# jmloveyj/ros_navigation

Measured on AMD Instinct MI355X. Metric: replan cycles/sec (HIMM+VFH++A*) on 4096x4096 grid, higher is better.
Workload: dtype int32; 1 GPU; full replan loop on 4096x4096 f32 grid (res 0.05 m); one step = one turn of the 20-stage A* pipeline = 20 passes of [100032-ray HIMM batch + fused compose -> 256 VFH+ poses -> 256 grid-A* queries (one launch)]; 30% rectangle obstacles (seed 2); 4 ray batches / pose sets / query sets in rotation; cycles_per_pass=256, rays_per_pass=100032, rotating_input_sets=4, astar_queries_checked=15360, astar_queries_answered=15360, astar_bucket_width=128000, astar_pipeline_depth=20, parallelism=query-sharded x1, full=False

## Files before the change

ros_navigation_amd/csrc/astar_tile.hip:

```cpp
#include "engine.hpp"
#include <algorithm>
#include <cstring>
#include <vector>

using namespace rna;

namespace rna {

constexpr int TI = 64, TJ = 16;
constexpr int TILE_WORDS = TI * TJ;
constexpr int AUX_WORDS = 64;
constexpr int MASK_STRIDE = TILE_WORDS + 32 + 128;
constexpr int TSA_WAVES = 8;
constexpr int TSA_WAVES_PER_EU = 8;
constexpr int TSA_HPASS = 4;
constexpr int TSA_IDLE_SLEEP = 4;
constexpr int TSA_PRIO_FIRST = 0;
constexpr int TSA_BT_PRIO = 3;
constexpr int TSA_SCOPE = __HIP_MEMORY_SCOPE_AGENT;
constexpr int TSA_MAX_TILE_WORDS = 2048;
constexpr int COST_S = 1000, COST_D = 1414;
constexpr int INF = 0x7fffffff;
constexpr int KU = 0x40000000;
constexpr int SCR_CNT = 84 + 192 + 48 + 64;
// ... 70 lines not shown

__device__ __forceinline__ int tile_of(int i, int j, int tiles_i) { return (j >> 4) * tiles_i + (i >> 6); }
__device__ __forceinline__ int in_page(int i, int j) { return ((j & 15) << 6) + (i & 63); }
__device__ __forceinline__ int kdi_of(int k) { return (k == 0 || k == 3 || k == 5) ? -1 : ((k == 2 || k == 4 || k == 7) ? 1 : 0); }
__device__ __forceinline__ int kdj_of(int k) { return k < 3 ? -1 : (k > 4 ? 1 : 0); }

struct TsaStage {
  unsigned* pages;
  unsigned* paux;
  unsigned* tmap;
  unsigned* owner;
  int* nalloc;
  uint8_t* nbr_tm;
  int* perm;
  int* ticket;
  int cap;
};
__host__ __device__ inline size_t tsa_align256(size_t x) { return (x + 255) & ~(size_t)255; }
constexpr int TSA_COUNTER_WORDS = 16;
__host__ __device__ inline unsigned long long* tsa_counters_of(const TsaStage& S) {
  return reinterpret_cast<unsigned long long*>(reinterpret_cast<char*>(S.nalloc) - TSA_COUNTER_WORDS * sizeof(unsigned long long));
}

__global__ void __launch_bounds__(256) tsa_snapshot_kernel(const uint8_t* __restrict__ nbr, int rows, int cols, int tiles_i, int tiles_j,
                                                             uint8_t* __restrict__ nbr_tm, int s0, int s1) {
  __shared__ unsigned s_free[256];
  const int a = threadIdx.x & 63, bq = threadIdx.x >> 6;
  for (int t = blockIdx.x; t < tiles_i * tiles_j; t += gridDim.x) {
    const int i = (t % tiles_i) * TI + a, j0 = (t / tiles_i) * TJ + bq * 4;
    unsigned v = 0u;
    if (i < rows) {
      const int bi = i + s0 >= rows ? i + s0 - rows : i + s0;
#pragma unroll
      for (int k = 0; k < 4; ++k)
        if (j0 + k < cols) {
          const int bj = j0 + k + s1 >= cols ? j0 + k + s1 - cols : j0 + k + s1;
          v |= (unsigned)nbr[(size_t)bj * rows + bi] << (8 * k);
        }
    }
    uint8_t* out = nbr_tm + (size_t)t * MASK_STRIDE;
    reinterpret_cast<unsigned*>(out)[a * 4 + bq] = v;
    if (a == 0) reinterpret_cast<unsigned*>(out + TILE_WORDS)[bq] = v;
    if (a == TI - 1) reinterpret_cast<unsigned*>(out + TILE_WORDS + 16)[bq] = v;
    s_free[threadIdx.x] = (((v & 0xffu) != 0u) ? 1u : 0u) | (((v & 0xff00u) != 0u) ? 2u : 0u) | (((v & 0xff0000u) != 0u) ? 4u : 0u) |
                          (((v & 0xff000000u) != 0u) ? 8u : 0u);
    __syncthreads();
    if (bq == 0)
      reinterpret_cast<unsigned short*>(out + TILE_WORDS + 32)[a] =
          (unsigned short)(s_free[a] | (s_free[64 + a] << 4) | (s_free[128 + a] << 8) | (s_free[192 + a] << 12));
    __syncthreads();
  }
}
__global__ void __launch_bounds__(256) tsa_prepare_kernel(TsaStage S, const rna_astar_query* __restrict__ queries, int n, int rows, int cols,
                                                          int ranked, int* __restrict__ served) {
  extern __shared__ int s_key[];
  if (threadIdx.x == 0) *S.ticket = 0;
  if (served && threadIdx.x < TSA_RETRY) served[threadIdx.x] = -1;
  if (served && threadIdx.x == TSA_RETRY) served[TSA_RETRY] = 0;
  if (!ranked) {
    for (int i = threadIdx.x; i < n; i += blockDim.x) S.perm[i] = i;
    return;
  }
  const int ncell = rows * cols;
  for (int i = threadIdx.x; i < n; i += blockDim.x) {
    const rna_astar_query q = queries[i];
    int key = -1;
    if (q.start >= 0 && q.goal >= 0 && q.start < ncell && q.goal < ncell) {
      const int di = abs(q.start % rows - q.goal % rows), dj = abs(q.start / rows - q.goal / rows);
      key = di > dj ? di : dj;
    }
    s_key[i] = key;
  }
  __syncthreads();
  for (int i = threadIdx.x; i < n; i += blockDim.x) {
    const int ki = s_key[i];
    int rank = 0;
    for (int j = 0; j < n; ++j) {
      const int kj = s_key[j];
      rank += (kj > ki || (kj == ki && j < i)) ? 1 : 0;
    }
    S.perm[rank] = i;
  }
}
__global__ void tsa_fill_pages_kernel(uint4* __restrict__ p, size_t n4) {
  const size_t step = (size_t)gridDim.x * blockDim.x;
  for (size_t w = (size_t)blockIdx.x * blockDim.x + threadIdx.x; w < n4; w += step) p[w] = make_uint4(0u, 0u, 0u, 0u);
}

#ifdef RNA_TSA_STATS
__device__ unsigned long long g_tsa_stat[32];
#define TSA_T(var) const unsigned long long var = wall_clock64()
#define TSA_ACC(slot, t0, t1) tsa_acc[slot] += (unsigned long long)((t1) - (t0))
#define TSA_CNT(slot, v) tsa_acc[slot] += (unsigned long long)(v)
#define TSA_ACC_PARAM , unsigned long long* tsa_acc
#define TSA_ACC_ARG , tsa_acc
#else
#define TSA_ACC_PARAM
#define TSA_ACC_ARG
#define TSA_T(var)
#define TSA_ACC(slot, t0, t1)
#define TSA_CNT(slot, v)
#endif

constexpr int TSA_NCLS = 256;
constexpr int TSA_NP = 3072;
constexpr int TSA_BMW = TSA_NP / 32;
constexpr int TSA_QC = 1024;
constexpr unsigned POP_EMPTY = 0xffffffffu;
static_assert(TSA_NP % 32 == 0 && TSA_NP < 0xffff, "node indices are 16 bits, 0xffff = none");
static_assert(TSA_NP * 4 >= (TI + 2) * (TJ + 2) * 4 + TILE_WORDS, "the backtrace's LDS image lives in the queue memory");

__device__ __forceinline__ unsigned lds_ld(const unsigned* p) { return __hip_atomic_load(p, __ATOMIC_RELAXED, __HIP_MEMORY_SCOPE_WORKGROUP); }
__device__ __forceinline__ int lds_ldi(const int* p) { return __hip_atomic_load(p, __ATOMIC_RELAXED, __HIP_MEMORY_SCOPE_WORKGROUP); }

struct TsaLocalSched {
  int* best_;
  int* state_;
  unsigned* st2_;
  unsigned* far_;
  unsigned* node_;
  unsigned* head_;
  unsigned* bm_;
  unsigned* qc_;
  int* count_;
  int* spill_;
  unsigned* open_;
  int* open_left_;
  __device__ __forceinline__ int best() const { return __hip_atomic_load(best_, __ATOMIC_RELAXED, __HIP_MEMORY_SCOPE_WORKGROUP); }
  __device__ __forceinline__ void improve_best(int g) { atomicMin(best_, g); }
  __device__ __forceinline__ void overflow() { *state_ = 4; }
  __device__ __forceinline__ void pool_exhausted() { *state_ = 5; }
  __device__ __forceinline__ void act_far(int t) { atomicOr(&far_[t >> 5], 1u << (t & 31)); }
  __device__ __forceinline__ bool is_far(int t) const { return (lds_ld(&far_[t >> 5]) >> (t & 31)) & 1u; }
  __device__ __forceinline__ int node_alloc(unsigned seed) {
    unsigned w = ((seed & 0xffffu) * (unsigned)TSA_BMW) >> 16;
    for (int tries = 0; tries < 32; ++tries) {
      const unsigned v = lds_ld(&bm_[w]);
      if (v) {
        const unsigned b = v & (0u - v);
        if (atomicAnd(&bm_[w], ~b) & b) return (int)(w * 32u) + __builtin_ctz(b);
      } else {
        w = w + 1u == (unsigned)TSA_BMW ? 0u : w + 1u;
      }
    }
    return -1;
  }
  __device__ __forceinline__ void node_free(int idx) { atomicOr(&bm_[idx >> 5], 1u << (idx & 31)); }
  __device__ __forceinline__ void link(int idx, unsigned t, unsigned cls) {
    for (;;) {
      const unsigned hv = lds_ld(&head_[cls]);
      __hip_atomic_store(&node_[idx], (hv << 16) | t, __ATOMIC_RELAXED, __HIP_MEMORY_SCOPE_WORKGROUP);
      asm volatile("" ::: "memory");
      if (atomicCAS(&head_[cls], hv, ((hv + 0x10000u) & 0xffff0000u) | (unsigned)idx) == hv) break;
    }
  }
  __device__ __forceinline__ void push(unsigned t, unsigned cls, int lane, int* spare) {
    if (lane == 0) {
      const int idx = *spare >= 0 ? *spare : node_alloc(t * 29u);
      if (idx >= 0) {
        link(idx, t, cls);
        atomicAdd(count_, 1);
        __hip_atomic_store(&qc_[t & (unsigned)(TSA_QC - 1)], (t << 8) | cls, __ATOMIC_RELAXED, __HIP_MEMORY_SCOPE_WORKGROUP);
      } else {
        atomicOr(&far_[t >> 5], 1u << (t & 31));
        *spill_ = 1;
      }
    }
    *spare = -1;
  }
// ... 436 lines not shown
                \
      unsigned long long hsrc_ = up_ & __builtin_amdgcn_ballot_w64(m_ > (mv_ & open_));                          \
      asm volatile("" : "+s"(hsrc_));           \
      const int ht_ = TSA_HT(b);                                                 \
      TSA_G(b) = max(TSA_G(b), m_);                                                                              \
      TSA_PP(b) = TSA_G(b) >= ht_ ? TSA_G(b) : 0;                                                                \
                                                            \
      unsigned left_ = 1u << (TSA_HPASS - 1);                                                                  \
      {                                                                                                          \
        int t1_, t2_;                                                                                            \
        asm volatile(                                                                                            \
            "s_nop 1\n"         \
            ".Lhp_top%=:\n\t"                                                                                     \
            "v_add_u32_dpp %[t1], %[pp], %[nS] wave_shr:1 row_mask:0xf bank_mask:0xf bound_ctrl:1\n\t"             \
            "v_add_u32_dpp %[t2], %[pp], %[nS] wave_shl:1 row_mask:0xf bank_mask:0xf bound_ctrl:1\n\t"             \
            "v_max_i32 %[t1], %[t1], %[t2]\n\t"                                                                   \
            "v_and_b32 %[t1], %[t1], %[open]\n\t"                                                                 \
            "v_cmp_gt_i32 vcc, %[t1], %[g]\n\t"                                                                   \
            "s_cbranch_vccz .Lhp_done%=\n\t"                                                                      \
            "v_max_i32 %[g], %[g], %[t1]\n\t"                                                                     \
            "s_or_b64 %[all], %[all], vcc\n\t"                                                                    \
            "v_cmp_ge_i32 vcc, %[g], %[ht]\n\t"                                                                   \
            "s_nop 1\n\t"                                                                                         \
            "v_cndmask_b32 %[pp], 0, %[g], vcc\n\t"                                                               \
            "s_lshr_b32 %[left], %[left], 1\n\t"                                                                  \
            "s_cbranch_scc1 .Lhp_top%=\n\t"                                                                       \
            ".Lhp_done%=:"                                                                                        \
            : [g] "+v"(TSA_G(b)), [pp] "+v"(TSA_PP(b)), [all] "+s"(up_), [left] "+s"(left_),                       \
              [t1] "=&v"(t1_), [t2] "=&v"(t2_)                                                                   \
            : [nS] "v"(nS), [open] "v"(open_), [ht] "v"(ht_)                                                     \
            : "vcc", "scc");                                                                                     \
      }                                                                                                          \
      TSA_STAT_HP(left_);                                                                                        \
      if (TSA_UNLIKELY(left_ == 0u)) {    \
        if (scan_ok) {                                                                                           \
          TSA_CNT(14, 1);                                                                                        \
          up_ |= tsa_row_fixpoint(TSA_G(b), TSA_PP(b), open_, ht_, thr, lane);                                   \
        } else {                                                                                                 \
          AGVAR |= 1u << (b);                                                                                    \
        }                                                                                                        \
      }                                                                                                          \
      TSA_ROW_CHANGED(b, up_, DIR, hsrc_, left_)                                                                 \
    }                                                                                                            \
  }
#define TSA_DOWN(b) if ((nd >> (b)) & 1u) { nd &= ~(1u << (b)); TSA_ROW(b, TSA_VERT(b, TSA_CAT(TSA_DEC_, b), 0, 2), nu, 0) }
#define TSA_UP(b) if ((nu >> (b)) & 1u) { nu &= ~(1u << (b)); TSA_ROW(b, TSA_VERT(b, TSA_CAT(TSA_INC_, b), 5, 7), nd, 1) }
  for (;;) {
    if (nd != 0u) {
      if (nd & 0x000fu) {
        if (nd & 1u) { nd &= ~1u; TSA_ROW(0, 0, nu, 0) }
        TSA_DOWN(1) TSA_DOWN(2) TSA_DOWN(3)
      }
      if (nd & 0x00f0u) { TSA_DOWN(4) TSA_DOWN(5) TSA_DOWN(6) TSA_DOWN(7) }
      if (nd & 0x0f00u) { TSA_DOWN(8) TSA_DOWN(9) TSA_DOWN(10) TSA_DOWN(11) }
      if (nd & 0xf000u) { TSA_DOWN(12) TSA_DOWN(13) TSA_DOWN(14) TSA_DOWN(15) }
    }
    if (!(nd | nu)) break;
    if (nu != 0u) {
      if (nu & 0xf000u) {
        if ((nu >> 15) & 1u) { nu &= ~(1u << 15); TSA_ROW(15, 0, nd, 1) }
        TSA_UP(14) TSA_UP(13) TSA_UP(12)
      }
      if (nu & 0x0f00u) { TSA_UP(11) TSA_UP(10) TSA_UP(9) TSA_UP(8) }
      if (nu & 0x00f0u) { TSA_UP(7) TSA_UP(6) TSA_UP(5) TSA_UP(4) }
      if (nu & 0x000fu) { TSA_UP(3) TSA_UP(2) TSA_UP(1) TSA_UP(0) }
    }
    if (!(nd | nu)) break;
  }
#undef TSA_DOWN
#undef TSA_UP
#undef TSA_ROW
#undef TSA_VERT
#undef TSA_STAT_INC
#undef TSA_STAT_HP
  TSA_T(t_c);
  TSA_ACC(1, t_b, t_c);
  TSA_CNT(8, evals);
  TSA_CNT(11, hpass);
  if (first) { TSA_CNT(18, 1); TSA_CNT(19, evals); TSA_CNT(20, __builtin_popcount(rowchg)); }
  TSA_CNT(21, __builtin_popcount(rowchg));
  asm volatile("; TSA_MARK results_begin");
  asm volatile("" : "+v"(lane));
  if (rowchg) {
    if (TSA_UNLIKELY(pg == 0u)) {
      int p = 0;
      if (lane == 0) {
        p = atomicAdd(C.nalloc, 1) + 1;
        if (p > C.cap) { p = 0; sch.pool_exhausted(); }
        else { C.owner[p] = (unsigned)t; __hip_atomic_store(&C.tmap[t], (unsigned)p, __ATOMIC_RELAXED, TSA_SCOPE); }
      }
      pg = (unsigned)__builtin_amdgcn_readfirstlane(p);
      if (pg == 0u) return;
    }
    unsigned* own = C.pages + (pg << 10);
    unsigned* ax = C.paux + pg * AUX_WORDS + (lane ? 16 : 0);
    const bool edge_lane = __builtin_amdgcn_inverse_ballot_w64(0x8000000000000001ull);
    const bool ovf_possible = lim_u > (unsigned)(KU - 5 * COST_D);
    unsigned long long ovfm = 0ull;
    const unsigned ulane = (unsigned)lane & 63u;
#define TSA_STORE(b) if ((rowchg >> (b)) & 1u) own[(b) * TI + ulane] = (unsigned)TSA_G(b);
    TSA_R16(TSA_STORE)
#undef TSA_STORE
    if (TSA_UNLIKELY(ovf_possible)) {
      unsigned rowchg_o = rowchg;
      asm volatile("" : "+s"(rowchg_o));
#define TSA_OVF(b) if ((rowchg_o >> (b)) & 1u) ovfm |= __builtin_amdgcn_ballot_w64((unsigned)(TSA_G(b) - 1) < (unsigned)(4 * COST_D - 1));
      TSA_R16(TSA_OVF)
#undef TSA_OVF
    }
    if (edge_lane) {
      uint4* a4 = reinterpret_cast<uint4*>(ax);
      a4[0] = make_uint4((unsigned)g0, (unsigned)g1, (unsigned)g2, (unsigned)g3);
      a4[1] = make_uint4((unsigned)g4, (unsigned)g5, (unsigned)g6, (unsigned)g7);
      a4[2] = make_uint4((unsigned)g8, (unsigned)g9, (unsigned)g10, (unsigned)g11);
      a4[3] = make_uint4((unsigned)g12, (unsigned)g13, (unsigned)g14, (unsigned)g15);
    }
    if (ovfm && lane == 0) sch.overflow();
    if (TSA_UNLIKELY(t == C.tg)) {
      unsigned rowchg_g = rowchg & (1u << C.gb);
      asm volatile("" : "+s"(rowchg_g));
#define TSA_GOAL(b)                                                                               \
  if ((rowchg_g >> (b)) & 1u) {                                                    \
    const int u = __builtin_amdgcn_readlane(TSA_G(b), C.ga);            \
    if (u != 0 && lane == 0) sch.improve_best(KU - u);                                            \
  }
      TSA_R16(TSA_GOAL)
#undef TSA_GOAL
    }
  }
  TSA_T(t_w0);
  asm volatile("; TSA_MARK wake_begin");
  {
    unsigned look = first ? 0xffffu : rowchg;
    asm volatile("" : "+s"(look));
    if (look && best1 > bucket_end && !sch.is_far(t)) {
      unsigned long long farm = 0ull;
      if (!TSA_UNLIKELY(best_in != INF)) {
        int acc = 0;
#define TSA_END(b) if ((look >> (b)) & 1u) acc |= TSA_G(b) ^ TSA_PP(b);
        TSA_R16(TSA_END)
#undef TSA_END
        farm = __builtin_amdgcn_ballot_w64(acc != 0);
      } else {
        const int thr_best = KU - best_in;
#define TSA_END(b)                                                                                               \
  if ((look >> (b)) & 1u) farm |= __builtin_amdgcn_ballot_w64(TSA_G(b) != 0 && TSA_PP(b) == 0 && TSA_G(b) >= TSA_HC(b, thr_best));
        TSA_R16(TSA_END)
#undef TSA_END
      }
      if (farm && lane == 0) sch.act_far(t);
    }
    if (TSA_UNLIKELY(first)) {
      q0 |= __builtin_amdgcn_ballot_w64(pp0 != 0);
      q15 |= __builtin_amdgcn_ballot_w64(pp15 != 0);
      qany |= (1ull << 63) | 1ull;
    }
    const bool col_any = (qany & 1ull) || (qany >> 63) || (q0 & 1ull) || (q0 >> 63) || (q15 & 1ull) || (q15 >> 63);
    bool wakeN = q0 != 0ull, wakeS = q15 != 0ull;
    int kfN = 0, kfS = 0, kfW = 0, kfE = 0;
    if (wakeN) {
      const int topv = (int)scr[84 + lane];
      const int c_ = __builtin_amdgcn_inverse_ballot_w64(q0) ? g0 : 0;
      const int cw_ = c_ & __builtin_amdgcn_sbfe((int)mk0, 0, 1), cn_ = c_ & __builtin_amdgcn_sbfe((int)mk0, 1, 1), ce_ = c_ & __builtin_amdgcn_sbfe((int)mk0, 2, 1);
      const int from_w_ = lane_m1(ce_) + nD, from_e_ = lane_p1(cw_) + nD;
      const int un_ = max3i(cn_ + nS, from_w_, from_e_);
      const bool imp_ = un_ > topv;
      wakeN = __builtin_amdgcn_ballot_w64(imp_) != 0ull;
      if (wakeN) kfN = wave_max_i32(imp_ ? un_ - TSA_H(-1) : (int)0x80000000);
    }
    if (wakeS) {
      const int botv = (int)scr[84 + 64 + lane];
      const int c_ = __builtin_amdgcn_inverse_ballot_w64(q15) ? g15 : 0;
      const int cw_ = c_ & __builtin_amdgcn_sbfe((int)mk3, 24 + 5, 1), cs_ = c_ & __builtin_amdgcn_sbfe((int)mk3, 24 + 6, 1), ce_ = c_ & __builtin_amdgcn_sbfe((int)mk3, 24 + 7, 1);
      const int from_w_ = lane_m1(ce_) + nD, from_e_ = lane_p1(cw_) + nD;
      const int un_ = max3i(cs_ + nS, from_w_, from_e_);
      const bool imp_ = un_ > botv;
      wakeS = __builtin_amdgcn_ballot_w64(imp_) != 0ull;
      if (wakeS) kfS = wave_max_i32(imp_ ? un_ - TSA_H(TJ) : (int)0x80000000);
    }
    unsigned colw = 0u;
    if (col_any) {
      if (__builtin_amdgcn_inverse_ballot_w64(0x8000000000000001ull)) {
        uint4* cp = reinterpret_cast<uint4*>(&scr[276 + (lane ? 32 : 0)]);
        cp[0] = make_uint4((unsigned)pp0, (unsigned)pp1, (unsigned)pp2, (unsigned)pp3);
        cp[1] = make_uint4((unsigned)pp4, (unsigned)pp5, (unsigned)pp6, (unsigned)pp7);
        cp[2] = make_uint4((unsigned)pp8, (unsigned)pp9, (unsigned)pp10, (unsigned)pp11);
        cp[3] = make_uint4((unsigned)pp12, (unsigned)pp13, (unsigned)pp14, (unsigned)pp15);
      }
      __builtin_amdgcn_wave_barrier();
      const int xl_ = lane & 31;
      const bool xr_ = lane >= 32;
      const int v_ = (xl_ >= 1 && xl_ <= TJ) ? (int)scr[276 + (lane & 32) + xl_ - 1] : 0;
      const int xv = (int)scr[84 + 128 + lane];
      const unsigned eb_ = scr[84 + 192 + 48 + lane];
      const int vs_ = v_ & -(int)((eb_ >> (xr_ ? 4 : 3)) & 1u), vu_ = v_ & -(int)((eb_ >> (xr_ ? 2 : 0)) & 1u), vd_ = v_ & -(int)((eb_ >> (xr_ ? 7 : 5)) & 1u);
      const int from_below_ = lane_p1(vu_) + nD, from_above_ = lane_m1(vd_) + nD;
      const int ux_ = max3i(vs_ + nS, from_below_, from_above_);
      const bool imp = (xl_ <= TJ + 1) & (ux_ > xv);
// ... 165 lines not shown
  if (lane == 0) A.results[q] = rna_astar_result{0, len, r.cost, r.expanded, r.rounds, r.buckets};
}

template <int WAVES, bool RETRY>
__global__ void __launch_bounds__(WAVES * 64) __attribute__((amdgpu_waves_per_eu(TSA_WAVES_PER_EU, TSA_WAVES_PER_EU))) tsa_search_kernel(const TsaLaunch A) {
  constexpr int TSA_THREADS = WAVES * 64;
  __shared__ __attribute__((aligned(16))) unsigned s_scr[WAVES][SCR_WORDS];
  extern __shared__ unsigned s_dyn[];
  __shared__ __attribute__((aligned(16))) unsigned s_node[TSA_NP];
  __shared__ __attribute__((aligned(16))) unsigned s_head[TSA_NCLS];
  __shared__ unsigned s_bm[TSA_BMW];
  __shared__ unsigned s_qc[TSA_QC];
  __shared__ int s_best, s_state, s_bucket, s_bucket0, s_jobs_done, s_jobs_noop, s_jobs_sticky, s_expanded, s_nalloc, s_any;
  __shared__ int s_count, s_spill, s_idle, s_open_left, s_open_pos, s_reruns;

  __shared__ int s_q, s_rank;
  if (!RETRY) {
    if (threadIdx.x == 0) { const int k = atomicAdd(A.S.ticket, 1); s_rank = k; s_q = A.S.perm[k]; }
  } else {
    if (threadIdx.x == 0) { s_q = A.retry_list[A.retry_base + (int)blockIdx.x]; s_rank = 1 << 30; }
  }
  __syncthreads();
  const int q = __builtin_amdgcn_readfirstlane(s_q);
  if (q < 0) return;
  if (RETRY && threadIdx.x == 0) A.S2.ticket[8 + blockIdx.x] = q;
  const TsaStage& S = RETRY ? A.S2 : A.S;
  const int sl = RETRY ? (int)blockIdx.x : q;
  if (__builtin_amdgcn_readfirstlane(s_rank) < A.prio_first) __builtin_amdgcn_s_setprio(3);
  const int tid = threadIdx.x, lane = tid & 63, wv = __builtin_amdgcn_readfirstlane(tid >> 6);
#ifdef RNA_TSA_STATS
  const unsigned long long t_kernel0 = wall_clock64();
#endif
  const int rows = A.rows, cols = A.cols, tiles_i = A.tiles_i, tiles_j = A.tiles_j;
  rna_astar_query qu = A.queries[q];
  const int ncell = rows * cols;
  const int ntile = tiles_i * tiles_j;
  const int nt_words = (ntile + 31) >> 5;
  unsigned* const s_st2 = s_dyn;
  unsigned* const s_open = s_dyn + 2 * nt_words;
  unsigned* const s_far = s_dyn + 3 * nt_words;
  rna_astar_result* const results = A.results;

  const bool valid = qu.start >= 0 && qu.goal >= 0 && qu.start < ncell && qu.goal < ncell;
  if (!valid) {
    if (tid == 0) results[q] = rna_astar_result{2, 0, INF, 0, 0, 0};
    return;
  }
  qu.start = tsa_unwrap_lin(qu.start, rows, cols, A.s0, A.s1);
  qu.goal = tsa_unwrap_lin(qu.goal, rows, cols, A.s0, A.s1);
  const int si = qu.start % rows, sj = qu.start / rows;
  const int gi = qu.goal % rows, gj = qu.goal / rows;

  TsaCtx C;
  C.rows = rows; C.cols = cols; C.tiles_i = tiles_i; C.tiles_j = tiles_j;
  C.tiles_magic = tiles_i > 1 ? (unsigned)(0x100000000ull / (unsigned)tiles_i) + 1u : 0u;
  C.pages = S.pages + (((size_t)sl * ((size_t)S.cap + 1)) << 10);
  C.paux = S.paux + (size_t)sl * ((size_t)S.cap + 1) * AUX_WORDS;
  C.tmap = S.tmap + (size_t)sl * ntile;
  C.owner = S.owner + (size_t)sl * (S.cap + 1);
  C.cap = S.cap;
  C.nalloc = &s_nalloc;
  C.nbr_tm = S.nbr_tm;
  C.gi = gi; C.gj = gj;
  C.ts = tile_of(si, sj, tiles_i); C.sa = si & (TI - 1); C.sb = sj & (TJ - 1);
  C.tg = tile_of(gi, gj, tiles_i); C.ga = gi & (TI - 1); C.gb = gj & (TJ - 1);

  for (int w = tid; w < 4 * nt_words; w += TSA_THREADS) s_dyn[w] = 0u;
  for (int w = tid; w < TSA_NCLS; w += TSA_THREADS) s_head[w] = 0xffffu;
  for (int w = tid; w < TSA_BMW; w += TSA_THREADS) s_bm[w] = 0xffffffffu;
  for (int w = tid; w < TSA_QC; w += TSA_THREADS) s_qc[w] = 0xffffffffu;
  if (lane >= 48) s_scr[wv][68 + lane - 48] = 0u;
  if (lane < 4) s_scr[wv][SCR_CNT + lane] = 0u;
  {
    const unsigned ms = C.nbr_tm[(size_t)C.ts * MASK_STRIDE + C.sa * 16 + C.sb], mg = C.nbr_tm[(size_t)C.tg * MASK_STRIDE + C.ga * 16 + C.gb];
    if (qu.goal != qu.start && (mg == 0u || ms == 0u)) {
      if (tid == 0) results[q] = rna_astar_result{1, 0, INF, 0, 0, 0};
      return;
    }
  }
  {
    const int used_raw = S.nalloc[sl];
    const int used = used_raw < C.cap ? used_raw : C.cap;
    if (used > 0) {
      uint4* pg4 = reinterpret_cast<uint4*>(C.pages + (1 << 10));
      for (size_t w = tid; w < (size_t)used * (TILE_WORDS / 4); w += TSA_THREADS) pg4[w] = make_uint4(0u, 0u, 0u, 0u);
      uint4* ax4 = reinterpret_cast<uint4*>(C.paux + AUX_WORDS);
      for (size_t w = tid; w < (size_t)used * (AUX_WORDS / 4); w += TSA_THREADS) ax4[w] = make_uint4(0u, 0u, 0u, 0u);
      for (int p = 1 + tid; p <= used; p += TSA_THREADS) C.tmap[C.owner[p]] = 0u;
      asm volatile("s_waitcnt vmcnt(0)" ::: "memory");
    }
  }
  int key_shift = 0;
  while (((long long)A.bucket_width >> key_shift) > TSA_NCLS - 1) ++key_shift;
  if (tid == 0) {
    s_best = INF; s_state = 0; s_jobs_done = 0; s_jobs_noop = 0; s_jobs_sticky = 0; s_expanded = 0; s_nalloc = 0;
    s_bucket = tsa_octile(si, sj, gi, gj) / A.bucket_width;
    s_bucket0 = s_bucket;
    s_spill = 0; s_idle = 0; s_open_pos = 0; s_reruns = 0;
    s_count = 1; s_open_left = 1;
  }
  __syncthreads();
  if (tid == 0) s_open[C.ts >> 5] = 1u << (C.ts & 31);
  __syncthreads();

#ifdef RNA_TSA_STATS
  unsigned long long tsa_acc[24] = {};
  const unsigned long long t_life0 = wall_clock64();
  const unsigned long long c_life0 = __builtin_amdgcn_s_memtime();
#endif
  TsaLocalSched sch{&s_best, &s_state, s_st2, s_far, s_node, s_head, s_bm, s_qc, &s_count, &s_spill, s_open, &s_open_left};
  int spare = -1;

  for (;;) {
    const int bucket = __builtin_amdgcn_readfirstlane(lds_ldi(&s_bucket));
    const long long bucket_end = ((long long)bucket + 1) * A.bucket_width;
    const unsigned bucket_end_u = bucket_end > 0x80000000LL ? 0x80000000u : (unsigned)bucket_end;
    const long long key_base_ll = (long long)KU - (long long)bucket * A.bucket_width;
    const int key_base = key_base_ll < -(long long)INF ? -INF : (int)key_base_ll;
    bool idle = false;
    bool open_blocked = false;
    for (;;) {
      TSA_T(t_p0);
      if (lds_ldi(&s_state) >= 4) break;
      if (idle) {
        if (lds_ldi(&s_idle) == WAVES) break;
        if (lds_ldi(&s_count) <= 0) { __builtin_amdgcn_s_sleep(TSA_IDLE_SLEEP); continue; }
        if (lane == 0) atomicSub(&s_idle, 1);
        idle = false;
      }
      int t = -1;
      int first = 0;
      const int open_left = lds_ldi(&s_open_left);
      if (!open_blocked && open_left > 0) {
        const int pos = lds_ldi(&s_open_pos);
        const unsigned w = pos + lane < nt_words ? lds_ld(&s_open[pos + lane]) : 0u;
        const unsigned long long nz = __builtin_amdgcn_ballot_w64(w != 0u);
        if (!nz) {
          if (lane == 0) atomicCAS(&s_open_pos, pos, pos + 64 >= nt_words ? 0 : pos + 64);
          continue;
        }
        const int l0 = __builtin_ctzll(nz);
        const unsigned w0 = (unsigned)__builtin_amdgcn_readlane((int)w, l0);
        const int b0 = __builtin_ctz(w0);
        const int tt = ((pos + l0) << 5) + b0;
        const unsigned sh = 2u * ((unsigned)tt & 15u);
        int r = 0;
        if (lane == 0) {
          if ((atomicAnd(&s_open[pos + l0], ~(1u << b0)) >> b0) & 1u) {
            const unsigned old = atomicOr(&s_st2[tt >> 4], 2u << sh) >> sh;
            if (old & 2u) {
              atomicOr(&s_open[pos + l0], 1u << b0);
              atomicOr(&s_st2[tt >> 4], 1u << sh);
              r = 2;
            } else {
              atomicAnd(&s_st2[tt >> 4], ~(1u << sh));
              atomicSub(&s_open_left, 1);
              atomicSub(&s_count, 1);
              r = 1;
            }
          }
        }
        r = __builtin_amdgcn_readfirstlane(r);
        if (r == 0) continue;
        if (r == 2) { open_blocked = true; continue; }
        t = tt;
        first = 1;
      } else {
        open_blocked = false;
        const unsigned e = sch.pop(lane, &spare);
        if (e == POP_EMPTY) {
// ... 126 lines not shown
  __syncthreads();
  const rna_astar_result r = results[q];
  int cnt = 0;
  if (r.status == 0 || r.status == 3) {
    const int goal = tsa_unwrap_lin(queries[q].goal, rows, cols, s0, s1);
    const int gi = goal % rows, gj = goal / rows;
    const int used = S.nalloc[sl];
    for (size_t w = threadIdx.x; w < ((size_t)used << 10); w += blockDim.x) {
      const int p = 1 + (int)(w >> 10), l = (int)(w & 1023);
      const int t = (int)S.owner[(size_t)sl * (S.cap + 1) + p];
      const int i = (t % tiles_i) * TI + (l & (TI - 1)), j = (t / tiles_i) * TJ + (l >> 6);
      const unsigned u = S.pages[(((size_t)sl * ((size_t)S.cap + 1) + p) << 10) + l];
      if (u != 0u && i < rows && j < cols && (KU - (int)u) + tsa_octile(i, j, gi, gj) <= r.cost) ++cnt;
    }
  }
  atomicAdd(&s_cnt, cnt);
  __syncthreads();
  if (threadIdx.x == 0) counts[q] = s_cnt;
}

static inline int tsa_ntile(const rna_engine* e) {
  return ((e->geom.size[0] + TI - 1) / TI) * ((e->geom.size[1] + TJ - 1) / TJ);
}
bool tsa_supported(const rna_engine* e) { return (size_t)tsa_ntile(e) <= (size_t)TSA_MAX_TILE_WORDS * 32; }
int tsa_tiles(const rna_engine* e) { return tsa_ntile(e); }
size_t tsa_pool_bytes(int max_queries, int cap) { return (size_t)max_queries * ((size_t)cap + 1) * (TILE_WORDS + AUX_WORDS) * sizeof(unsigned); }
size_t tsa_aux_bytes(const rna_engine* e, int max_queries, int cap) {
  const size_t ntile = (size_t)tsa_ntile(e);
  return 256 + 2 * tsa_align256((size_t)max_queries * sizeof(int)) + tsa_align256(ntile * MASK_STRIDE) +
         tsa_align256((size_t)max_queries * ntile * sizeof(unsigned)) + tsa_align256((size_t)max_queries * ((size_t)cap + 1) * sizeof(unsigned));
}
static TsaStage tsa_stage_view(const rna_engine* e, int slot) {
  const AstarDevice& a = e->astar;
  const size_t ntile = (size_t)tsa_ntile(e);
  char* base = static_cast<char*>(a.tsa_aux[slot]);
  TsaStage S;
  S.cap = a.page_cap;
  S.pages = reinterpret_cast<unsigned*>(a.g[slot]);
  S.paux = S.pages + (((size_t)a.max_queries * ((size_t)S.cap + 1)) << 10);
  S.ticket = reinterpret_cast<int*>(base);
  base += 256;
  S.nalloc = reinterpret_cast<int*>(base);
  base += tsa_align256((size_t)a.max_queries * sizeof(int));
  S.perm = reinterpret_cast<int*>(base);
  base += tsa_align256((size_t)a.max_queries * sizeof(int));
  S.nbr_tm = reinterpret_cast<uint8_t*>(base);
  base += tsa_align256(ntile * MASK_STRIDE);
  S.tmap = reinterpret_cast<unsigned*>(base);
  base += tsa_align256((size_t)a.max_queries * ntile * sizeof(unsigned));
  S.owner = reinterpret_cast<unsigned*>(base);
  return S;
}
size_t tsa_retry_pool_bytes(const rna_engine* e) { return tsa_pool_bytes(TSA_RETRY, tsa_ntile(e)); }
size_t tsa_retry_aux_bytes(const rna_engine* e) {
  const size_t ntile = (size_t)tsa_ntile(e);
  return 256 + tsa_align256(TSA_RETRY * sizeof(int)) + tsa_align256((size_t)TSA_RETRY * ntile * sizeof(unsigned)) +
         tsa_align256((size_t)TSA_RETRY * (ntile + 1) * sizeof(unsigned)) + tsa_align256((size_t)e->astar.max_queries * sizeof(int));
}
static int* tsa_retry_list(const rna_engine* e, int slot) {
  const size_t ntile = (size_t)tsa_ntile(e);
  return reinterpret_cast<int*>(static_cast<char*>(e->astar.tsa_aux_retry[slot]) + 256 + tsa_align256(TSA_RETRY * sizeof(int)) +
                                tsa_align256((size_t)TSA_RETRY * ntile * sizeof(unsigned)) + tsa_align256((size_t)TSA_RETRY * (ntile + 1) * sizeof(unsigned)));
}
static int* tsa_retry_served(const rna_engine* e, int slot) { return reinterpret_cast<int*>(e->astar.tsa_aux_retry[slot]) + 8; }
static int* tsa_retry_count(const rna_engine* e, int slot) { return tsa_retry_served(e, slot) + TSA_RETRY; }
static TsaStage tsa_retry_view(const rna_engine* e, int slot, const TsaStage& main) {
  const AstarDevice& a = e->astar;
  const size_t ntile = (size_t)tsa_ntile(e);
  char* base = static_cast<char*>(a.tsa_aux_retry[slot]);
  TsaStage S = main;
  S.cap = (int)ntile;
  S.pages = reinterpret_cast<unsigned*>(a.g_retry[slot]);
  S.paux = S.pages + (((size_t)TSA_RETRY * ((size_t)S.cap + 1)) << 10);
  S.ticket = reinterpret_cast<int*>(base);
  base += 256;
  S.nalloc = reinterpret_cast<int*>(base);
  base += tsa_align256(TSA_RETRY * sizeof(int));
  S.tmap = reinterpret_cast<unsigned*>(base);
  base += tsa_align256((size_t)TSA_RETRY * ntile * sizeof(unsigned));
  S.owner = reinterpret_cast<unsigned*>(base);
  return S;
}
int tsa_retry_prepare(rna_engine* e, int slot) {
  hipLaunchKernelGGL(tsa_fill_pages_kernel, dim3(2048), dim3(256), 0, e->stream, reinterpret_cast<uint4*>(e->astar.g_retry[slot]),
                     tsa_retry_pool_bytes(e) / sizeof(uint4));
  RNA_HIP(e, hipGetLastError());
  return RNA_OK;
}
int tsa_stage_prepare(rna_engine* e, int slot) {
  const TsaStage S = tsa_stage_view(e, slot);
  const size_t pages = (size_t)e->astar.max_queries * ((size_t)S.cap + 1);
  hipLaunchKernelGGL(tsa_fill_pages_kernel, dim3(8192), dim3(256), 0, e->stream, reinterpret_cast<uint4*>(S.pages),
                     pages * (TILE_WORDS + AUX_WORDS) / 4);
  RNA_HIP(e, hipGetLastError());
  return RNA_OK;
}

size_t tsa_ring_bytes(const rna_engine* e, int max_queries) {
  return 256 + tsa_align256((size_t)max_queries * sizeof(int)) + tsa_align256((size_t)tsa_ntile(e) * MASK_STRIDE);
}
static_assert(sizeof(TsaLaunch) <= sizeof(AstarDevice::last_launch[0]), "AstarDevice::last_launch holds a TsaLaunch");

int tsa_retry_launch(rna_engine* e, int slot, hipStream_t search_stream, int count) {
  AstarDevice& a = e->astar;
  TsaLaunch A;
  memcpy(&A, a.last_launch[slot], sizeof(A));
  A.retry = 1;
  A.retry_count = nullptr;
  A.S2 = tsa_retry_view(e, slot, A.S);
  for (int base = 0; base < count; base += TSA_RETRY) {
    A.retry_base = base;
    const int wgs = std::min(TSA_RETRY, count - base);
    if (a.depth > 1) hipLaunchKernelGGL((tsa_search_kernel<TSA_WAVES, true>), dim3(wgs), dim3(TSA_WAVES * 64), a.last_lds[slot], search_stream, A);
    else hipLaunchKernelGGL((tsa_search_kernel<16, true>), dim3(wgs), dim3(16 * 64), a.last_lds[slot], search_stream, A);
    RNA_HIP(e, hipGetLastError());
  }
  return RNA_OK;
}

int tsa_launch(rna_engine* e, int slot, hipStream_t init_stream, hipStream_t search_stream, hipEvent_t ev_init,
               const rna_astar_query* q_dev, int n, int32_t* paths_dev, int max_len, rna_astar_result* res_dev) {
  AstarDevice& a = e->astar;
  const int rows = e->geom.size[0], cols = e->geom.size[1];
  const int ti = (rows + TI - 1) / TI, tj = (cols + TJ - 1) / TJ;
  TsaStage S = tsa_stage_view(e, slot);
  hipStream_t prep_stream = search_stream;
  int ring = -1;
  if (ev_init) {
    ring = (int)(a.launches % (unsigned long long)a.ring_n);
    char* base = a.ring_mem + (size_t)ring * a.ring_stride;
    S.ticket = reinterpret_cast<int*>(base);
    S.perm = reinterpret_cast<int*>(base + 256);
    S.nbr_tm = reinterpret_cast<uint8_t*>(base + 256 + tsa_align256((size_t)a.max_queries * sizeof(int)));
    { const int rc = side_stream(e, &prep_stream); if (rc != RNA_OK) return rc; }
    RNA_HIP(e, hipEventRecord(ev_init, init_stream));
    RNA_HIP(e, hipStreamWaitEvent(prep_stream, ev_init, 0));
    if (a.ring_used[ring]) RNA_HIP(e, hipStreamWaitEvent(prep_stream, a.ring_free[ring], 0));
  }
  {
    KernelTimer kt(e, RNA_K_ASTAR_INIT, prep_stream);
    hipLaunchKernelGGL(tsa_snapshot_kernel, dim3(std::min(ti * tj, 4096)), dim3(256), 0, prep_stream, e->nbr, rows, cols, ti, tj, S.nbr_tm,
                       e->geom.start[0], e->geom.start[1]);
    RNA_HIP(e, hipGetLastError());
  }
  if (ev_init) {
    RNA_HIP(e, hipEventRecord(a.snap_done[slot], prep_stream));
    a.snap_pending[slot] = true;
  }
  {
    KernelTimer kt(e, RNA_K_ASTAR_RESET, prep_stream);
    const int ranked = n <= 2048 ? 1 : 0;
    hipLaunchKernelGGL(tsa_prepare_kernel, dim3(1), dim3(256), ranked ? (size_t)n * sizeof(int) : 0, prep_stream, S, q_dev, n, rows, cols, ranked,
                       a.g_retry[slot] ? tsa_retry_served(e, slot) : nullptr);
    RNA_HIP(e, hipGetLastError());
  }
  if (ev_init) {
    RNA_HIP(e, hipEventRecord(a.ev_prep, prep_stream));
    RNA_HIP(e, hipStreamWaitEvent(search_stream, a.ev_prep, 0));
  }
  {
    KernelTimer kt(e, RNA_K_ASTAR_SEARCH, search_stream);
    const size_t nt_bytes = (size_t)((ti * tj + 31) / 32) * sizeof(unsigned);
    TsaLaunch A;
    memset(&A, 0, sizeof(A));
    A.rows = rows; A.cols = cols; A.tiles_i = ti; A.tiles_j = tj; A.s0 = e->geom.start[0]; A.s1 = e->geom.start[1];
    A.queries = q_dev; A.S = S; A.bucket_width = a.bucket_width; A.paths = paths_dev; A.max_path_len = max_len;
    A.rev_all = a.rev[slot]; A.rev_cap = a.rev_cap; A.results = res_dev;
    A.retry = 0; A.n = n; A.S2 = S;
    A.prio_first = a.depth > 1 ? TSA_PRIO_FIRST : 0;
    if (const char* pf = getenv("RNA_TSA_PRIO_FIRST")) A.prio_first = atoi(pf);
    size_t lds_dyn = 4 * nt_bytes;
    if (const char* pad = getenv("RNA_TSA_LDS_PAD")) lds_dyn += (size_t)atoi(pad);
    const bool can_retry = a.g_retry[slot] != nullptr && a.retry_flag != nullptr;
    A.retry_count = can_retry ? tsa_retry_count(e, slot) : nullptr;
    A.retry_list = can_retry ? tsa_retry_list(e, slot) : nullptr;
    A.retry_base = 0;
// ... 80 lines not shown
```

Before: 168,200 replan cycles/s.

## Write full tile on first page allocation instead of zero-filling page pools

Drops the bulk zero-fill of every page in the stage and retry pools, and the per-query clearing of used pages at the start of a search. Instead, when a tile page is freshly allocated, all 16 rows are written, and the tile map entry is published only after those stores complete. Only page 0 of each query region is still zeroed, by a small kernel. This saves a lot of memory bandwidth per replan, at the cost of a wait on memory before publishing the map entry and a reliance on fresh pages never being read before their first full write (aux words included).

```diff
diff --git a/ros_navigation_amd/csrc/astar_tile.hip b/ros_navigation_amd/csrc/astar_tile.hip
--- a/ros_navigation_amd/csrc/astar_tile.hip
+++ b/ros_navigation_amd/csrc/astar_tile.hip
@@ -176,9 +176,11 @@
     S.perm[rank] = i;
   }
 }
-__global__ void tsa_fill_pages_kernel(uint4* __restrict__ p, size_t n4) {
-  const size_t step = (size_t)gridDim.x * blockDim.x;
-  for (size_t w = (size_t)blockIdx.x * blockDim.x + threadIdx.x; w < n4; w += step) p[w] = make_uint4(0u, 0u, 0u, 0u);
+__global__ void __launch_bounds__(256) tsa_zero_page0_kernel(unsigned* __restrict__ pages, unsigned* __restrict__ paux, int cap) {
+  static_assert(TILE_WORDS / 4 == 256 && AUX_WORDS / 4 <= 256, "one uint4 of page 0 per thread");
+  const size_t page0 = (size_t)blockIdx.x * ((size_t)cap + 1);
+  reinterpret_cast<uint4*>(pages + (page0 << 10))[threadIdx.x] = make_uint4(0u, 0u, 0u, 0u);
+  if (threadIdx.x < AUX_WORDS / 4) reinterpret_cast<uint4*>(paux + page0 * AUX_WORDS)[threadIdx.x] = make_uint4(0u, 0u, 0u, 0u);
 }
 
 #ifdef RNA_TSA_STATS
@@ -781,23 +783,27 @@
   asm volatile("; TSA_MARK results_begin");
   asm volatile("" : "+v"(lane));
   if (rowchg) {
+    unsigned fresh = 0u;
     if (TSA_UNLIKELY(pg == 0u)) {
       int p = 0;
       if (lane == 0) {
         p = atomicAdd(C.nalloc, 1) + 1;
         if (p > C.cap) { p = 0; sch.pool_exhausted(); }
-        else { C.owner[p] = (unsigned)t; __hip_atomic_store(&C.tmap[t], (unsigned)p, __ATOMIC_RELAXED, TSA_SCOPE); }
+        else C.owner[p] = (unsigned)t;
       }
       pg = (unsigned)__builtin_amdgcn_readfirstlane(p);
       if (pg == 0u) return;
-    }
+      fresh = 1u;
+    }
+    unsigned rowchg_store = fresh ? 0xffffu : rowchg;
+    asm volatile("" : "+s"(rowchg_store));
     unsigned* own = C.pages + (pg << 10);
     unsigned* ax = C.paux + pg * AUX_WORDS + (lane ? 16 : 0);
     const bool edge_lane = __builtin_amdgcn_inverse_ballot_w64(0x8000000000000001ull);
     const bool ovf_possible = lim_u > (unsigned)(KU - 5 * COST_D);
     unsigned long long ovfm = 0ull;
     const unsigned ulane = (unsigned)lane & 63u;
-#define TSA_STORE(b) if ((rowchg >> (b)) & 1u) own[(b) * TI + ulane] = (unsigned)TSA_G(b);
+#define TSA_STORE(b) if ((rowchg_store >> (b)) & 1u) own[(b) * TI + ulane] = (unsigned)TSA_G(b);
     TSA_R16(TSA_STORE)
 #undef TSA_STORE
     if (TSA_UNLIKELY(ovf_possible)) {
@@ -813,6 +819,10 @@
       a4[1] = make_uint4((unsigned)g4, (unsigned)g5, (unsigned)g6, (unsigned)g7);
       a4[2] = make_uint4((unsigned)g8, (unsigned)g9, (unsigned)g10, (unsigned)g11);
       a4[3] = make_uint4((unsigned)g12, (unsigned)g13, (unsigned)g14, (unsigned)g15);
+    }
+    if (TSA_UNLIKELY(fresh)) {
+      asm volatile("s_waitcnt vmcnt(0)" ::: "memory");
+      if (lane == 0) __hip_atomic_store(&C.tmap[t], pg, __ATOMIC_RELAXED, TSA_SCOPE);
     }
     if (ovfm && lane == 0) sch.overflow();
     if (TSA_UNLIKELY(t == C.tg)) {
@@ -1144,10 +1154,6 @@
     const int used_raw = S.nalloc[sl];
     const int used = used_raw < C.cap ? used_raw : C.cap;
     if (used > 0) {
-      uint4* pg4 = reinterpret_cast<uint4*>(C.pages + (1 << 10));
-      for (size_t w = tid; w < (size_t)used * (TILE_WORDS / 4); w += TSA_THREADS) pg4[w] = make_uint4(0u, 0u, 0u, 0u);
-      uint4* ax4 = reinterpret_cast<uint4*>(C.paux + AUX_WORDS);
-      for (size_t w = tid; w < (size_t)used * (AUX_WORDS / 4); w += TSA_THREADS) ax4[w] = make_uint4(0u, 0u, 0u, 0u);
       for (int p = 1 + tid; p <= used; p += TSA_THREADS) C.tmap[C.owner[p]] = 0u;
       asm volatile("s_waitcnt vmcnt(0)" ::: "memory");
     }
@@ -1440,16 +1446,14 @@
   return S;
 }
 int tsa_retry_prepare(rna_engine* e, int slot) {
-  hipLaunchKernelGGL(tsa_fill_pages_kernel, dim3(2048), dim3(256), 0, e->stream, reinterpret_cast<uint4*>(e->astar.g_retry[slot]),
-                     tsa_retry_pool_bytes(e) / sizeof(uint4));
+  const TsaStage S = tsa_retry_view(e, slot, tsa_stage_view(e, slot));
+  hipLaunchKernelGGL(tsa_zero_page0_kernel, dim3(TSA_RETRY), dim3(256), 0, e->stream, S.pages, S.paux, S.cap);
   RNA_HIP(e, hipGetLastError());
   return RNA_OK;
 }
 int tsa_stage_prepare(rna_engine* e, int slot) {
   const TsaStage S = tsa_stage_view(e, slot);
-  const size_t pages = (size_t)e->astar.max_queries * ((size_t)S.cap + 1);
-  hipLaunchKernelGGL(tsa_fill_pages_kernel, dim3(8192), dim3(256), 0, e->stream, reinterpret_cast<uint4*>(S.pages),
-                     pages * (TILE_WORDS + AUX_WORDS) / 4);
+  hipLaunchKernelGGL(tsa_zero_page0_kernel, dim3(e->astar.max_queries), dim3(256), 0, e->stream, S.pages, S.paux, S.cap);
   RNA_HIP(e, hipGetLastError());
   return RNA_OK;
 }
```

Result: faster. 172,800 replan cycles/s, median of 6 (+2.7%).
